# latk/hbetune.rs

Hardware: AMD Instinct MI355X
Metric: GP fit+predict/sec (n=4096,d=8,f64) (higher is better)
Workload: dtype f64; 1 GPU; M: rosenbrock d=8 n=4096 f64, Matern nu=5/2 x constant + white noise; fixed-work fit = 3 L-BFGS runs x 150 lml+gradient evaluations + K^-1, then predict mean+variance at m=1600; evals_per_fit=450, n_not_pd=0, m_candidates=1600, parallelism=replicas x1 (independent fits per GPU, no collective)

## Files before the change

### csrc/dag_kernel.inc.hpp

```cpp

template <typename T, int TA, int TB>
struct DagGeom {
  using C = Cfg<T>;
  static constexpr int NT = 512;
  static constexpr int BK = C::BK;
  static constexpr int SK = BK + 2;
  static constexpr int SMA = TA + 16, SMB = TB + 16;
  static constexpr int LDSA = (TA * SK > BK * SMA) ? TA * SK : BK * SMA;
  static constexpr int LDSB = (TB * SK > BK * SMB) ? TB * SK : BK * SMB;
  static constexpr int NCHA = TA * BK / C::VEC / NT, NCHB = TB * BK / C::VEC / NT;
  static constexpr int WM = 4, WN = 2;
  static constexpr int TMA = TA / WM / 16, TMB = TB / WN / 16;
  static_assert(NCHA >= 1 && NCHB >= 1 && TMA >= 1 && TMB >= 1, "tile too small for 512 threads");
};

constexpr int DAG_LDS_CTL_OFF = (int)((LeafGeom<double>::LDS_BYTES + 15) / 16 * 16);
constexpr int DAG_LDS_BYTES = DAG_LDS_CTL_OFF + 128;
static_assert(DAG_LDS_BYTES <= 163840, "the diagonal block and the control words must fit the CU's LDS");

template <typename T, int TA, int TB, typename PullFn, typename FetchFn>
__device__ __forceinline__ void dag_gemm_tile(int flags, int row0, int col0, int kbeg, int kend, T* __restrict__ W1,
                                              T* __restrict__ W2, T* __restrict__ W3, T* __restrict__ Kinv, int ld, char* smem_raw,
                                              PullFn pull, FetchFn fetch, unsigned long long* inner = nullptr) {
  using C = Cfg<T>;
  using G = DagGeom<T, TA, TB>;
  using vec_t = typename C::vec_t;
  using acc_t = typename C::acc_t;
  constexpr int VEC = C::VEC, BK = G::BK, SK = G::SK, SMA = G::SMA, SMB = G::SMB, NCHA = G::NCHA, NCHB = G::NCHB;
  constexpr int TMA = G::TMA, TMB = G::TMB, NT = G::NT;

  const int akm = (flags & DAGF_AKM) ? 1 : 0, bkm = (flags & DAGF_BKM) ? 1 : 0;
  const T* Ag = (flags & DAGF_A3) ? W3 : ((flags & DAGF_ABUF) ? W2 : W1);
  const T* Bg = (flags & DAGF_B3) ? W3 : ((flags & DAGF_BBUF) ? W2 : W1);
  T* Cg = (flags & DAGF_CKINV) ? Kinv : ((flags & DAGF_C3) ? W3 : ((flags & DAGF_CBUF) ? W2 : W1));
  const int nstages = (kend - kbeg) / BK;

  T* lds = reinterpret_cast<T*>(smem_raw);
  const int t = threadIdx.x, lane = t & 63, wave = t >> 6;
  const int wm = wave >> 1, wn = wave & 1;

  constexpr int CPK = BK / VEC;
  constexpr int RPP_K = NT / CPK;
  constexpr int CPRA = TA / VEC, CPRB = TB / VEC;
  constexpr int RPP_MA = NT / CPRA, RPP_MB = NT / CPRB;
  const int a_r0 = akm ? t / CPRA : t / CPK, a_c0 = akm ? (t % CPRA) * VEC : (t % CPK) * VEC;
  const int b_r0 = bkm ? t / CPRB : t / CPK, b_c0 = bkm ? (t % CPRB) * VEC : (t % CPK) * VEC;
  const int a_rpp = akm ? RPP_MA : RPP_K, b_rpp = bkm ? RPP_MB : RPP_K;
  const int a_lds0 = a_r0 * (akm ? SMA : SK) + a_c0, a_ldsq = a_rpp * (akm ? SMA : SK);
  const int b_lds0 = 2 * G::LDSA + b_r0 * (bkm ? SMB : SK) + b_c0, b_ldsq = b_rpp * (bkm ? SMB : SK);

  const T* pA = Ag + (akm ? (size_t)(kbeg + a_r0) * ld + row0 + a_c0 : (size_t)(row0 + a_r0) * ld + kbeg + a_c0);
  const T* pB = Bg + (bkm ? (size_t)(kbeg + b_r0) * ld + col0 + b_c0 : (size_t)(col0 + b_r0) * ld + kbeg + b_c0);
  const size_t a_step = akm ? (size_t)BK * ld : (size_t)BK, b_step = bkm ? (size_t)BK * ld : (size_t)BK;
  const size_t a_qs = (size_t)a_rpp * ld, b_qs = (size_t)b_rpp * ld;

  vec_t ra0[NCHA], rb0[NCHB], ra1[NCHA], rb1[NCHB];
  auto load_stage = [&](vec_t (&ra)[NCHA], vec_t (&rb)[NCHB]) {
#pragma unroll
    for (int q = 0; q < NCHA; ++q) ra[q] = *reinterpret_cast<const vec_t*>(pA + q * a_qs);
#pragma unroll
    for (int q = 0; q < NCHB; ++q) rb[q] = *reinterpret_cast<const vec_t*>(pB + q * b_qs);
    pA += a_step;
    pB += b_step;
  };
  auto store_stage = [&](int buf, vec_t (&ra)[NCHA], vec_t (&rb)[NCHB]) {
#pragma unroll
    for (int q = 0; q < NCHA; ++q) C::lds_store(lds + buf * G::LDSA + a_lds0 + q * a_ldsq, ra[q]);
#pragma unroll
    for (int q = 0; q < NCHB; ++q) C::lds_store(lds + buf * G::LDSB + b_lds0 + q * b_ldsq, rb[q]);
  };

  acc_t acc[TMA][TMB];
// ... 47 lines not shown
#pragma unroll
      for (int a = 0; a < TMA; ++a)
#pragma unroll
        for (int b = 0; b < TMB; ++b) {
#pragma unroll
          for (int r = 0; r < 4; ++r) tot[a][b][r] += (double)acc[a][b][r];
          acc[a][b] = acc_t{0, 0, 0, 0};
          if constexpr (TA * TB >= 128 * 128) __builtin_amdgcn_sched_barrier(0);
        }
    }
  };

  const int soA = akm ? 1 : SK, skA = akm ? SMA : 1;
  const int soB = bkm ? 1 : SK, skB = bkm ? SMB : 1;
  const int fa0 = (wm * (TA / G::WM) + (lane & 15)) * soA + (lane >> 4) * skA;
  const int fb0 = 2 * G::LDSA + (wn * (TB / G::WN) + (lane & 15)) * soB + (lane >> 4) * skB;

  constexpr int NK = BK / 4;
  T fa[NK][TMA], fb[NK][TMB];
  auto read_frags = [&](int buf, int k4) {
    const int ia = buf * G::LDSA + fa0 + k4 * 4 * skA, ib = buf * G::LDSB + fb0 + k4 * 4 * skB;
#pragma unroll
    for (int a = 0; a < TMA; ++a) fa[k4][a] = lds[ia + a * 16 * soA];
#pragma unroll
    for (int b2 = 0; b2 < TMB; ++b2) fb[k4][b2] = lds[ib + b2 * 16 * soB];
  };
  auto mfma_step = [&](int k4) {
#pragma unroll
    for (int a = 0; a < TMA; ++a)
#pragma unroll
      for (int b2 = 0; b2 < TMB; ++b2) acc[a][b2] = C::mfma(fa[k4][a], fb[k4][b2], acc[a][b2]);
  };
  auto stage = [&](int cur, bool do_load, vec_t (&la)[NCHA], vec_t (&lb)[NCHB], bool do_store, vec_t (&sa)[NCHA],
                   vec_t (&sb)[NCHB], bool has_next) {
    if (do_load) load_stage(la, lb);
    constexpr bool SPLIT_READS = NK >= 8 && TA * TB >= 128 * 128;
    constexpr int KH = SPLIT_READS ? NK / 2 : NK - 1;
#pragma unroll
    for (int k4 = 1; k4 <= KH; ++k4) read_frags(cur, k4);
    if constexpr (SPLIT_READS) {
#pragma unroll
      for (int k4 = 0; k4 + 1 < KH; ++k4) mfma_step(k4);
      __builtin_amdgcn_sched_barrier(0);
#pragma unroll
      for (int k4 = KH + 1; k4 < NK; ++k4) read_frags(cur, k4);
#pragma unroll
      for (int k4 = KH - 1; k4 + 2 < NK; ++k4) mfma_step(k4);
    } else {
#pragma unroll
      for (int k4 = 0; k4 + 2 < NK; ++k4) mfma_step(k4);
    }
    __builtin_amdgcn_sched_barrier(0);
    if (do_store) store_stage(cur ^ 1, sa, sb);
    if (NK >= 2) mfma_step(NK - 2);
    __builtin_amdgcn_sched_barrier(0);
    __syncthreads();
    __builtin_amdgcn_sched_barrier(0);
    if (has_next) read_frags(cur ^ 1, 0);
    mfma_step(NK - 1);
    __builtin_amdgcn_sched_group_barrier(0x100, TMA + TMB, 0);
    __builtin_amdgcn_sched_group_barrier(0x008, TMA * TMB, 0);
    __builtin_amdgcn_sched_barrier(0);
    kabs += BK;
    if (CHUNKED && kabs % F32_CHUNK == 0) flush();
  };
  if (nstages > 0) {
    load_stage(ra0, rb0);
    if (nstages > 1) load_stage(ra1, rb1);
    if constexpr (!PREFETCH_C && !NOACC) {
      if (accum) {
        T cst[TMA][TMB][4];
        const int er0p = row0 + wm * (TA / G::WM), ec0p = col0 + wn * (TB / G::WN) + (lane & 15);
#pragma unroll
        for (int a = 0; a < TMA; ++a)
#pragma unroll
          for (int b = 0; b < TMB; ++b)
#pragma unroll
            for (int r = 0; r < 4; ++r) cst[a][b][r] = Cg[(size_t)(er0p + a * 16 + C::crow(lane, r)) * ld + ec0p + b * 16];
        store_stage(0, ra0, rb0);
        bool stash = true;
        if constexpr (sizeof(T) == 8) {
          if (cinit) {
            stash = false;
#pragma unroll
            for (int a = 0; a < TMA; ++a)
#pragma unroll
              for (int b = 0; b < TMB; ++b)
#pragma unroll
                for (int r = 0; r < 4; ++r) acc[a][b][r] = cst[a][b][r];
          }
        }
        if (stash) {
#pragma unroll
          for (int a = 0; a < TMA; ++a)
#pragma unroll
            for (int b = 0; b < TMB; ++b)
#pragma unroll
              for (int r = 0; r < 4; ++r) lds[STASH_OFF + ((a * TMB + b) * 4 + r) * NT + t] = cst[a][b][r];
        }
      } else {
        store_stage(0, ra0, rb0);
      }
    } else {
      store_stage(0, ra0, rb0);
    }
    __syncthreads();
    read_frags(0, 0);
#ifdef DAG_STAMP_INNER
    unsigned long long st1 = 0;
    if (inner && t == 0) st1 = __builtin_amdgcn_s_memrealtime();
#endif
    int s = 0;
    for (; s + 3 < nstages; s += 2) {
      stage(0, true, ra0, rb0, true, ra1, rb1, true);
      stage(1, true, ra1, rb1, true, ra0, rb0, true);
    }
    const int left = nstages - s;
    if (left <= 2) pull();
    if (left == 1) fetch();
    stage(0, left > 2, ra0, rb0, left > 1, ra1, rb1, left > 1);
    if (left > 2) pull();
    if (left == 2) fetch();
    if (left > 1) stage(1, false, ra1, rb1, left > 2, ra0, rb0, left > 2);
    if (left > 2) {
      fetch();
      stage(0, false, ra0, rb0, false, ra1, rb1, false);
    }
#ifdef DAG_STAMP_INNER
    if (inner && t == 0) *inner = ((st1 & 0xffffffffull) << 32) | (__builtin_amdgcn_s_memrealtime() & 0xffffffffull);
#endif
  } else {
    pull();
    fetch();
  }

  flush();
  const int er0 = row0 + wm * (TA / G::WM), ec0 = col0 + wn * (TB / G::WN) + (lane & 15);
  const bool neg = (flags & DAGF_NEG) != 0;
  T cend[NOACC ? TMA : 1][NOACC ? TMB : 1][4];
  if constexpr (NOACC) {
    if (accum) {
#pragma unroll
      for (int a = 0; a < TMA; ++a)
#pragma unroll
        for (int b = 0; b < TMB; ++b)
#pragma unroll
          for (int r = 0; r < 4; ++r) cend[a][b][r] = Cg[(size_t)(er0 + a * 16 + C::crow(lane, r)) * ld + ec0 + b * 16];
    }
  }
#pragma unroll
  for (int a = 0; a < TMA; ++a)
#pragma unroll
    for (int b = 0; b < TMB; ++b)
#pragma unroll
      for (int r = 0; r < 4; ++r) {
        const int row = er0 + a * 16 + C::crow(lane, r);
        T* p = Cg + (size_t)row * ld + ec0 + b * 16;
        T v;
        if constexpr (CHUNKED) v = (T)tot[a][b][r];
// ... 178 lines not shown
    const int kind = kf & 0xffff, flags = (kf >> 16) & 0xffff;
    const int row0 = __builtin_amdgcn_readfirstlane(ctl[5]), col0 = __builtin_amdgcn_readfirstlane(ctl[6]);
    const int kbeg = __builtin_amdgcn_readfirstlane(ctl[7]), kend = __builtin_amdgcn_readfirstlane(ctl[8]);
    const int sig0 = (__builtin_amdgcn_readfirstlane(ctl[9]) >> 16) & 0xffff, sig12 = __builtin_amdgcn_readfirstlane(ctl[10]);
    const int sig1 = sig12 & 0xffff, sig2 = (sig12 >> 16) & 0xffff;
    const int this_idx = __builtin_amdgcn_readfirstlane(ctl[0]);
    int ndesc = 0, nidx = 0;
    bool pulled = false, fetched = false;
    auto pull = [&]() {
      if (t == 0) nxt = __hip_atomic_fetch_add(g.ctrl, 1, __ATOMIC_RELAXED, __HIP_MEMORY_SCOPE_AGENT);
      pulled = true;
    };
    auto fetch = [&]() {
      if (t < 64) {
        nidx = __builtin_amdgcn_readfirstlane(nxt);
        if (nidx < g.ntasks && t < TASK_DW) ndesc = reinterpret_cast<const int*>(g.tasks + nidx)[t];
      }
      fetched = true;
    };
#ifdef DAG_STAMP_INNER
    unsigned long long* inner_stamp = g.trace ? g.trace + (size_t)this_idx * 5 + 4 : nullptr;
#else
    unsigned long long* inner_stamp = nullptr;
#endif
    if (status == 0) {
      if (kind == DAG_LEAF) {
        dag_leaf_task<T>(W1, W2, g.ld, row0, static_cast<T*>(g.ldiag), g.info, smem_raw, g.leaf_dbg & 16);
      } else if ((flags & DAGF_CKINV) && g.Kinv == nullptr) {
      } else if (kind == DAG_GEMM_128x64) {
        dag_gemm_tile<T, 128, 64>(flags, row0, col0, kbeg, kend, W1, W2, static_cast<T*>(g.W3), static_cast<T*>(g.Kinv), g.ld, smem_raw, pull, fetch, inner_stamp);
      } else if (kind == DAG_GEMM_64x64) {
        dag_gemm_tile<T, 64, 64>(flags, row0, col0, kbeg, kend, W1, W2, static_cast<T*>(g.W3), static_cast<T*>(g.Kinv), g.ld, smem_raw, pull, fetch, inner_stamp);
      } else if (kind == DAG_GEMM_128x128) {
        dag_gemm_tile<T, 128, 128>(flags, row0, col0, kbeg, kend, W1, W2, static_cast<T*>(g.W3), static_cast<T*>(g.Kinv), g.ld, smem_raw, pull, fetch, inner_stamp);
      } else if (kind == DAG_GEMM_32x64) {
        dag_gemm_tile_chain<T>(flags, row0, col0, kbeg, kend, W1, W2, static_cast<T*>(g.W3), g.ld, smem_raw, pull, fetch);
      }
    }
    if (!pulled) pull();
    if (!fetched) fetch();
    if (g.trace && t == 0) g.trace[(size_t)this_idx * 5 + 2] = __builtin_amdgcn_s_memrealtime();
    int* nctl = ctl_base + 16 * (par ^ 1);
    int look_c = 0, look_need = 0, look_inf = 0;
    const bool have_next = t < 64 && nidx < g.ntasks;
    if (have_next) look_issue(ndesc, &look_c, &look_need, &look_inf);
    asm volatile("s_waitcnt vmcnt(0)" ::: "memory");
    if (t < 64) {
      int nstatus = 2, early = 1;
      if (have_next) {
        const bool all_ok = __ballot(look_c < look_need) == 0ull;
        const int inf = __shfl(look_inf, 8, 64);
        if (inf < 0) {
          nstatus = 2;
        } else if (all_ok) {
          __builtin_amdgcn_fence(__ATOMIC_ACQUIRE, "agent");
          nstatus = inf > 0 ? 1 : 0;
          if (g.trace && t == 0) g.trace[(size_t)nidx * 5 + 0] = __builtin_amdgcn_s_memrealtime();
        } else {
          early = 0;
        }
      }
      if (early) {
        if (t < TASK_DW) nctl[4 + t] = ndesc;
        if (t == 0) {
          nctl[0] = nidx;
          nctl[1] = nstatus;
          asm volatile("s_waitcnt vmcnt(0)" ::: "memory");
// ... 44 lines not shown
```

### csrc/engine.hpp

```cpp
#pragma once
#include <hip/hip_runtime_api.h>
#include <cstddef>
#include <cstdint>

namespace hbegp {

constexpr int NB = 128;
constexpr int MAXD = 64;
constexpr int MAXP = MAXD + 2;

struct EvalParams {
  double noise;
  double amp;
  double ell[MAXD];
  unsigned long long seq;
};

struct EvalOut {
  double lml;
  double yalpha;
  double logdet;
  double grad[MAXP];
  int info;
  int n_warn;
// ... 43 lines not shown
  DAG_GEMM_32x64 = 8,
  DAG_GEMM_128x128 = 9,
};
enum : uint16_t {
  DAGF_ABUF = 1,
  DAGF_BBUF = 2,
  DAGF_CBUF = 4,
  DAGF_AKM = 8,
  DAGF_BKM = 16,
  DAGF_NEG = 32,
  DAGF_ACC = 64,
  DAGF_CKINV = 128,
  DAGF_A3 = 256,
  DAGF_B3 = 512,
  DAGF_C3 = 1024,
  DAGF_CINIT = 2048,
};
constexpr int DAG_MAXWAIT = 4;
constexpr int DAG_MAXSIG = 3;
constexpr uint16_t DAG_NOSIG = 0xffff;
struct DagTask {
  uint16_t kind, flags;
  int32_t row0, col0;
  int32_t kbeg, kend;
  uint16_t nwait;
  uint16_t sig[DAG_MAXSIG];
  uint16_t wcnt[DAG_MAXWAIT];
  uint16_t wval[DAG_MAXWAIT];
  uint16_t cost;
  uint16_t pad_[1];
};
static_assert(DAG_MAXSIG == 3, "DagTask::sig has three entries: dword 5 high half, dword 6 low half, dword 6 high half");
static_assert(sizeof(DagTask) == 48, "DagTask layout");
constexpr int DAG_CTRL_WORDS = 4;
constexpr int DAG_INFO_TIMEOUT = -2;
struct DagLaunch {
  const DagTask* tasks;
  int ntasks;
  int* ctrl;
  void* W1;
  void* W2;
  void* W3;
  void* Kinv;
  int ld;
  void* ldiag;
  int* info;
  unsigned long long* trace;
  unsigned long long wait_ticks;
  int leaf_dbg;
};
template <typename T>
void launch_dag(const DagLaunch& g, int nwg, hipStream_t s);
int dag_stage_depth(bool is_f32);

template <typename T>
void launch_gemm(const GemmLaunch& g, int tile, hipStream_t s);

template <typename T>
void launch_kmat(const T* X, const T* rv, int n, int d, int np, int nu2, const EvalParams* P, T* W, const int* info, hipStream_t s,
                 const EvalPrologue* pro = nullptr);

template <typename T>
void launch_leaf(T* W1, T* W2, int ld, int blk, T* ldiag, int* info, hipStream_t s, int dbg = 0);

template <typename T>
void launch_alpha_lml(const T* Xinv, int np, int n, const T* y, const T* ldiag, T* wbuf, double* part, T* alpha,
                      EvalOut* out, const int* info, hipStream_t s, int* ticket = nullptr);

template <typename T>
void launch_gradtrace(const T* X, int n, int d, int np, int nu2, const EvalParams* P, const T* Kinv, const T* alpha,
                      double* part, EvalOut* out, const int* info, hipStream_t s, int* ticket = nullptr, EvalOut* hout = nullptr);
size_t gradtrace_part_elems(int np, int d);

size_t loo_diag_part_elems(int np, int n);
size_t loo_u_part_elems(int np);
template <typename T>
void launch_loo_diag(const T* Xinv, int np, int n, const T* y, const T* alpha, double* part, T* mean, T* var, T* lpd, double* avec,
                     double* sbvec, EvalOut* out, hipStream_t s);
template <typename T>
void launch_loo_uy(const T* Kinv, int np, int n, const double* avec, const double* sbvec, T* Y, double* pu, T* u, hipStream_t s);
template <typename T>
void launch_loo_trace(const T* X, int n, int d, int np, int nu2, const EvalParams* P, const T* Cm, const T* alpha, const T* u,
// ... 176 lines not shown
```

### csrc/hbegp.cpp

```cpp
#include "../include/hbegp.h"

#include <hip/hip_runtime_api.h>

#include <algorithm>
#include <atomic>
#include <queue>
#include <cmath>
#include <cstdarg>
#include <cstdio>
#include <cstdlib>
#include <cstring>
#include <functional>
#include <limits>
#include <memory>
#include <mutex>
#include <numeric>
#include <string>
#include <thread>
#include <type_traits>
#include <vector>

#include "dag_plan.hpp"
#include "engine.hpp"
#include "lbfgsb.hpp"
// ... 664 lines not shown
  bool dag_rl_ = false;
  double dag_gflop_lauum = 0;
  struct DagVariant {
    int nwg = 0;
    std::vector<DagTask*> tasks;
    std::vector<DagTask> host_tasks;
    int nwg_p1 = 0, ntasks_p1 = 0, nwg_kinv = 0, ntasks_kinv = 0;
    std::vector<DagTask*> tasks_p1, tasks_kinv;
    std::vector<DagTask> host_tasks_p1, host_tasks_kinv;
  };
  std::vector<DagVariant> dag_var;
  std::unique_ptr<std::atomic<int>[]> busy_slots_;
  int dag_ntasks = 0, dag_nwg = 0;
  int dag_nvar_ = 1, dag_ncrowd_ = 0;
  int dag_nshare_ = 0;
  int share_hyst_ = SLOT_SHARE_HYSTERESIS;
  int slot_maxeval_ = 0;
  std::vector<int> share_force_;
  std::vector<char> balance_dev_;
  std::unique_ptr<std::atomic<int>[]> slot_running_, slot_done_;
  mutable std::atomic<int> not_alone_{0};
  unsigned long long dag_wait_ticks_ = 200000000ull;
  size_t dag_ctrl_bytes = 0;
  int dag_ctrl_regions_ = 1;
  double dag_gflop = 0;
  bool adhoc_ = false;
  bool small_ = false;
  bool like_fit_ = false;
  bool lazy_ = false;
  std::function<std::shared_ptr<const DagPlan>(int, bool, int)> plan_for_;
  bool hostio_ = true;
  bool eval_published() const { return hostio_ && !small_; }
  int leaf_dbg_ = 0;

  struct Pooled { int dev; void* p; size_t bytes; };
  std::vector<Pooled> pooled_;
  template <typename U>
  U* palloc(int dev, size_t count) {
    bool fresh = false;
    const size_t bytes = std::max<size_t>(16, sizeof(U) * count);
    void* q = g_pool.get(dev, bytes, &fresh);
    pooled_.push_back({dev, q, bytes});
    return static_cast<U*>(q);
  }

  Problem(hbegp_ctx* c, const T* X, const T* y, int n_, int d_, double nu, int n_slots_, bool single_shot = false, bool like_fit = false,
          bool lazy_fit = false, const double* rv = nullptr) {
    try {
      adhoc_ = single_shot;
      like_fit_ = like_fit;
      lazy_ = lazy_fit && env_int("HBEGP_LAZY_GRAD", 1) != 0;
      init(c, X, y, n_, d_, nu, n_slots_, rv);
    } catch (...) {
      release();
      throw;
    }
  }

  void init(hbegp_ctx* c, const T* X, const T* y, int n_, int d_, double nu, int n_slots_, const double* rv) {
    ctx = c; n = n_; d = d_; np = round_up(n_, NB); n_slots = n_slots_;
    nu2 = std::isinf(nu) ? 0 : (int)std::lround(2 * nu);
    is_f32 = sizeof(T) == 4;
    leaf_dbg_ = env_int("HBEGP_LEAF_DBG", 0) & 16;
    small_ = np == NB && d <= SMALL_EVAL_MAXD && env_int("HBEGP_SMALL", 1) != 0;
    hostio_ = env_int("HBEGP_HOSTIO", 1) != 0;
    lazy_ = lazy_ && eval_published() && !adhoc_;
    const size_t nn = (size_t)np * np;
    Xd.assign(c->devs.size(), nullptr);
    yd.assign(c->devs.size(), nullptr);
    rvd.assign(c->devs.size(), nullptr);
    std::vector<T> rv_t;
    if (rv) rv_t.assign(rv, rv + n_);
    slots.resize(c->devs.size());
    for (size_t di = 0; di < c->devs.size(); ++di) {
      HIPCHECK(hipSetDevice(c->devs[di]));
      slots[di].resize(n_slots);
      for (auto& s : slots[di]) {
        s.dev = c->devs[di];
        s.stream = g_stream_pool.get(s.dev);
      }
      hipStream_t st0 = slots[di][0].stream;
      Xd[di] = palloc<T>(c->devs[di], (size_t)n * d);
      yd[di] = palloc<T>(c->devs[di], np);
      HIPCHECK(hipMemsetAsync(yd[di], 0, sizeof(T) * np, st0));
      HIPCHECK(hipMemcpyAsync(Xd[di], X, sizeof(T) * (size_t)n * d, hipMemcpyHostToDevice, st0));
      HIPCHECK(hipMemcpyAsync(yd[di], y, sizeof(T) * n, hipMemcpyHostToDevice, st0));
      if (rv) {
        rvd[di] = palloc<T>(c->devs[di], n);
        HIPCHECK(hipMemcpyAsync(rvd[di], rv_t.data(), sizeof(T) * n, hipMemcpyHostToDevice, st0));
      }
      for (auto& s : slots[di]) {
        bool fresh1 = false, fresh2 = false, fk = false;
        s.W1 = static_cast<T*>(g_pool.get(s.dev, sizeof(T) * nn, &fresh1));
        s.W2 = static_cast<T*>(g_pool.get(s.dev, sizeof(T) * nn, &fresh2));
        for (int b = 0; b < 2; ++b) s.Kinv[b] = static_cast<T*>(g_pool.get(s.dev, sizeof(T) * nn, &fk));
        HIPCHECK(hipMemsetAsync(s.W2, 0, sizeof(T) * nn, st0));
// ... 355 lines not shown
    if (!s.dag_ctrl) return;
    std::vector<int> ctrl(dag_ctrl_bytes / sizeof(int));
    if (hipMemcpyAsync(ctrl.data(), s.dag_ctrl + (s.dag_part == 2 ? dag_ctrl_bytes / sizeof(int) : 0), dag_ctrl_bytes, hipMemcpyDeviceToHost, s.stream) != hipSuccess || hipStreamSynchronize(s.stream) != hipSuccess) return;
    const int row = ctrl[1] - 1;
    const DagVariant& var = dag_var[s.dag_variant];
    const int ntasks_here = s.dag_part == 1 ? var.ntasks_p1 : (s.dag_part == 2 ? var.ntasks_kinv : dag_ntasks);
    fprintf(stderr, "task queue timeout: queue head %d of %d, first task that gave up: %d\n", ctrl[0], ntasks_here, row);
    const std::vector<DagTask>& host_tasks = s.dag_part == 1 ? var.host_tasks_p1 : (s.dag_part == 2 ? var.host_tasks_kinv : var.host_tasks);
    if (row >= 0 && row < (int)host_tasks.size()) {
      const DagTask& t = host_tasks[row];
      fprintf(stderr, "  kind %d flags %x row0 %d col0 %d k [%d, %d) waits:", t.kind, t.flags, t.row0, t.col0, t.kbeg, t.kend);
      for (int w = 0; w < t.nwait; ++w) fprintf(stderr, " c%d=%d/%d", t.wcnt[w], ctrl[DAG_CTRL_WORDS + t.wcnt[w]], t.wval[w]);
      fprintf(stderr, "\n");
    }
    (void)hipGetLastError();
  }

  void launch_queue(Slot<T>& s, size_t di, T* Kinv, PhaseTimer* tm, int part = 0) {
    if (part != 2 && !s.ctrl_cleared) HIPCHECK(hipMemsetAsync(s.dag_ctrl, 0, dag_ctrl_regions_ * dag_ctrl_bytes, s.stream));
    if (part != 2) s.ctrl_cleared = false;
    DagLaunch g{};
    const DagVariant& var = dag_var[s.dag_variant];
    g.tasks = var.tasks[di]; g.ntasks = dag_ntasks; g.ctrl = s.dag_ctrl;
    int nwg = var.nwg;
    s.dag_part = part;
    if (part == 1) { g.tasks = var.tasks_p1[di]; g.ntasks = var.ntasks_p1; nwg = var.nwg_p1; }
    if (part == 2) { g.tasks = var.tasks_kinv[di]; g.ntasks = var.ntasks_kinv; nwg = var.nwg_kinv; g.ctrl = s.dag_ctrl + dag_ctrl_bytes / sizeof(int); }
    g.W1 = s.W1; g.W2 = s.W2; g.ld = np; g.ldiag = s.ldiag; g.info = &s.dOut->info;
    g.W3 = s.W3;
    g.Kinv = (dag_lauum_ && part != 1) ? Kinv : nullptr;
    g.trace = s.dag_trace;
    g.wait_ticks = dag_wait_ticks_;
    g.leaf_dbg = leaf_dbg_;
    if (tm) tm->begin(PhaseTimer::DAG, 0, part == 2 ? dag_gflop_lauum : (g.Kinv ? dag_gflop : dag_gflop - dag_gflop_lauum));
    launch_dag<T>(g, nwg, s.stream);
    if (tm) tm->end();
  }

  void small_eval(Slot<T>& s, size_t di, int target, int mode) {
    SmallEval g{};
    g.X = Xd[di]; g.y = yd[di]; g.n = n; g.d = d;
    g.W2 = s.W2; g.ldiag = s.ldiag; g.Kinv = s.Kinv[target]; g.alpha = s.alpha[target]; g.out = s.dOut; g.mode = mode;
    g.P = s.hP; g.hout = s.hOut;
    launch_small_eval<T>(g, rvd[di], nu2, s.stream);
  }

  enum EvalMode { EVAL_LML_KINV = 0, EVAL_FULL = 1, EVAL_LML_ONLY = 2, EVAL_GRAD_ONLY = 3 };

  void enqueue_eval(Slot<T>& s, size_t di, int target, int mode, PhaseTimer* tm) {
    const int* info = &s.dOut->info;
    const bool want_grad = mode == EVAL_FULL || mode == EVAL_GRAD_ONLY;
    if (mode == EVAL_GRAD_ONLY) {
      if (dag_ && dag_lauum_) launch_queue(s, di, s.Kinv[target], tm, 2);
      else eval_gemms(s, s.Kinv[target], scheduled(s, di, tm, (int)scheds[di].size() - 1), leaf_step(s, tm), [] {}, 2);
      const bool fuse_grad = (np / 64) * (np / 64 + 1) / 2 <= 512;
      if (tm) tm->begin(PhaseTimer::GRAD);
      launch_gradtrace<T>(Xd[di], n, d, np, nu2, s.dP, s.Kinv[target], s.alpha[target], s.part_g, s.dOut, info, s.stream,
                          fuse_grad ? s.tickets + 1 : nullptr, fuse_grad ? s.hOut : nullptr);
      if (tm) tm->end();
      if (!fuse_grad) launch_publish_out(s.dOut, s.hOut, s.dP, s.stream);
      s.published = true;
      CHECK_LAUNCHES();
      return;
    }
    const int part = mode == EVAL_LML_ONLY ? 1 : 0;
    if (small_) {
// ... 3866 lines not shown
int hbegp_debug_dag_replay(int nblocks, int bk, int small_h, int nwg, int order_wg, int fine, int big128, int which, int workers,
                           int* ntasks, int* tasks, int cap, double* out, char* err, int errlen) {
  if (nblocks < 1 || (bk != 16 && bk != 32) || small_h < 0 || nwg < 1 || which < 0 || which > 2 || !ntasks || workers < 0)
    return fail(HBEGP_EINVAL, "bad argument");
  GUARD_BEGIN
  DagBuilder builder(bk, small_h, nwg, (fine & 1) != 0, order_wg);
  builder.set_rl_progressive((fine & 16) != 0);
  builder.set_big128(big128 != 0, big128 >= 2);
  builder.set_rl(32, 1, (fine & 32) == 0, true);
  DagPlan plan = builder.build(0, nblocks, which != 1, (fine & 8) != 0);
  if (which == 2) plan = dag_plan_kinv_only(plan);
  const std::string why = plan.tasks.empty() ? std::string("no tasks") : dag_plan_validate(plan, nblocks);
  *ntasks = (int)plan.tasks.size();
  if (tasks)
    for (int i = 0; i < std::min(cap, (int)plan.tasks.size()); ++i) {
      const DagTask& t = plan.tasks[i];
      int* v = tasks + (size_t)18 * i;
      v[0] = t.kind; v[1] = t.flags; v[2] = t.row0; v[3] = t.col0; v[4] = t.kbeg; v[5] = t.kend; v[6] = t.nwait;
      for (int w = 0; w < DAG_MAXWAIT; ++w) { v[7 + w] = w < t.nwait ? t.wcnt[w] : 0; v[11 + w] = w < t.nwait ? t.wval[w] : 0; }
      for (int q = 0; q < DAG_MAXSIG; ++q) v[15 + q] = t.sig[q];
    }
  if (out) {
    const DagReplay r = workers > 0 ? dag_plan_replay(plan, workers) : DagReplay();
    double acc128 = 0;
    for (const DagTask& t : plan.tasks)
      if (t.kind == DAG_GEMM_128x128 && (t.flags & DAGF_ACC)) acc128 += t.cost * 0.1;
    out[0] = r.makespan_us; out[1] = r.wait_us; out[2] = r.busy_us; out[3] = plan.sim_us; out[4] = plan.crit_us; out[5] = acc128;
  }
  if (err && errlen > 0) snprintf(err, (size_t)errlen, "%s", why.c_str());
  return why.empty() ? HBEGP_OK : fail(HBEGP_EINVAL, "%s", why.c_str());
  GUARD_END
}

int hbegp_debug_dag_order_wg(int queue, int share, int nwg, int even_wg, int nblocks, int n_slots) {
  return dag_default_order_wg(queue, share, nwg, even_wg, nblocks, n_slots);
}

int hbegp_debug_lbfgs_replay(int n, const double* x0, const double* lo, const double* hi, int maxeval, int memory, int fixed_work,
                             int count, const double* f, const double* g, double* requested, int* n_requested) {
  if (n < 1 || n > LBFGS_MAXN || count < 0 || !x0 || !lo || !hi || !requested || !n_requested || (count > 0 && (!f || !g)))
    return fail(HBEGP_EINVAL, "bad argument");
  GUARD_BEGIN
  return lbfgs_replay_impl(n, x0, lo, hi, maxeval, memory, fixed_work, count, f, g, requested, nullptr, nullptr, nullptr, n_requested);
  GUARD_END
}

int hbegp_debug_dag_plan(int nblocks, int bk, int small_h, int nwg, int fine, int* ntasks, int* ncounters, int* nleaf,
                         double* gflop, double* crit_us, double* sim_us, char* err, int errlen) {
  if (nblocks < 1 || (bk != 16 && bk != 32) || small_h < 0 || nwg < 0) return fail(HBEGP_EINVAL, "bad argument");
  GUARD_BEGIN
  DagBuilder builder(bk, small_h, nwg, (fine & 1) != 0);
  builder.set_rl_progressive((fine & 16) != 0);
  builder.set_big128(getenv("HBEGP_DAG_BIG128") && atoi(getenv("HBEGP_DAG_BIG128")) != 0, getenv("HBEGP_DAG_BIG128") && atoi(getenv("HBEGP_DAG_BIG128")) >= 2);
  if (fine & 2) return fail(HBEGP_EINVAL, "fine bit 1 (kernel-matrix / reduction tasks in the queue) no longer exists");
  DagPlan plan = builder.build(0, nblocks, (fine & 4) != 0, (fine & 8) != 0);
  if (const char* fault = getenv("HBEGP_DAG_TEST_FAULT")) {
    int a = 0, b = 0;
    if (sscanf(fault, "drop:%d", &a) == 1 && a >= 0 && a < (int)plan.tasks.size() && plan.tasks[a].nwait > 0) {
      DagTask& t = plan.tasks[a];
      for (int w = 1; w < t.nwait; ++w) { t.wcnt[w - 1] = t.wcnt[w]; t.wval[w - 1] = t.wval[w]; }
      t.nwait--;
    } else if (sscanf(fault, "move:%d:%d", &a, &b) == 2 && a >= 0 && b >= 0 && a < (int)plan.tasks.size() && b < (int)plan.tasks.size()) {
      const DagTask t = plan.tasks[a];
      plan.tasks.erase(plan.tasks.begin() + a);
      plan.tasks.insert(plan.tasks.begin() + b, t);
    }
// ... 34 lines not shown
```

### hbetune_rs_amd/_lib.py

```python
import ctypes as C
import os

import numpy as np

HERE = os.path.dirname(os.path.abspath(__file__))
LIB_PATH = os.environ.get("HBEGP_LIB") or os.path.join(HERE, "libhbegp.so")

OK, NOT_PD, ALL_FAILED = 0, 1, 2
EINVAL, EHIP, ENODEV, ENOMEM = -1, -2, -3, -4
PATHS_MAX_FEATURES, PATHS_MAX_PATHS = 16384, 1024
CEI_MAX_CONSTRAINTS = 8
MES_MAX_SAMPLES = 1024
EHVI_ND_MAX_BOXES = 1048576
STATS_MAX_RUNS = 16


class HbegpError(RuntimeError):
    def __init__(self, code, msg):
        super().__init__(f"hbegp error {code}: {msg}")
        self.code = code


class FitOptions(C.Structure):

# ... 139 lines not shown
    "hbegp_paths_eval_f64": (C.c_int, [_vp, _dp, C.c_int, C.c_int, _dp, _dp]),
    "hbegp_paths_eval_f32": (C.c_int, [_vp, _fp, C.c_int, C.c_int, _fp, _fp]),
    "hbegp_paths_minimize_f64": (C.c_int, [_vp, _dp, C.c_int, _dp, _dp, C.c_int, _dp, _dp, _ip]),
    "hbegp_paths_minimize_f32": (C.c_int, [_vp, _fp, C.c_int, _dp, _dp, C.c_int, _fp, _dp, _ip]),
    "hbegp_paths_info": (C.c_int, [_vp, _ip, _ip, _ip, _ip, _ip]),
    "hbegp_paths_release": (None, [_vp]),
    "hbegp_debug_paths_phases": (C.c_int, [C.c_int, _dp]),
    "hbegp_debug_posterior_phases": (C.c_int, [C.c_int, _dp]),
    "hbegp_debug_batch_select_phases": (C.c_int, [C.c_int, _dp]),
    "hbegp_debug_kg_phases": (C.c_int, [C.c_int, _dp]),
    "hbegp_debug_nei_phases": (C.c_int, [C.c_int, _dp]),
    "hbegp_debug_sens_phases": (C.c_int, [C.c_int, _dp]),
    "hbegp_debug_ehvi_phases": (C.c_int, [C.c_int, _dp]),
    "hbegp_debug_ehvi_nd_phases": (C.c_int, [C.c_int, _dp]),
    "hbegp_debug_cei_phases": (C.c_int, [C.c_int, _dp]),
    "hbegp_debug_lcei_phases": (C.c_int, [C.c_int, _dp]),
    "hbegp_debug_mes_phases": (C.c_int, [C.c_int, _dp]),
    "hbegp_debug_cb_phases": (C.c_int, [C.c_int, _dp]),
    "hbegp_debug_pool_poisoned": (C.c_int, [C.POINTER(C.c_longlong), C.POINTER(C.c_longlong)]),
    "hbegp_model_info": (C.c_int, [_vp, _ip, _ip, _ip, _dp, _dp]),
    "hbegp_model_get_f64": (C.c_int, [_vp, _dp, _dp, _dp]),
    "hbegp_model_get_f32": (C.c_int, [_vp, _dp, _fp, _fp]),
    "hbegp_model_debug_params": (C.c_int, [_vp, _dp]),
    "hbegp_model_retain": (None, [_vp]),
    "hbegp_model_release": (None, [_vp]),
    "hbegp_debug_lbfgs_replay": (C.c_int, [C.c_int, _dp, _dp, _dp, C.c_int, C.c_int, C.c_int, C.c_int, _dp, _dp, _dp, _ip]),
    "hbegp_last_fit_stats": (C.c_int, [C.POINTER(FitStats)]),
    "hbegp_debug_lbfgs_decisions": (C.c_int, [C.c_int, _dp, _dp, _dp, C.c_int, C.c_int, C.c_int, C.c_int, _dp, _dp, _dp, _ip, _ip, _ip, _ip]),
    "hbegp_debug_dag_queues": (C.c_int, [C.c_int, C.c_int, C.c_int, C.c_int, C.c_int, C.c_int, C.c_int, _ip, _ip, C.c_int, C.c_char_p,
                                         C.c_int]),
    "hbegp_debug_dag_replay": (C.c_int, [C.c_int, C.c_int, C.c_int, C.c_int, C.c_int, C.c_int, C.c_int, C.c_int, C.c_int, _ip, _ip,
                                         C.c_int, _dp, C.c_char_p, C.c_int]),
    "hbegp_debug_dag_order_wg": (C.c_int, [C.c_int, C.c_int, C.c_int, C.c_int, C.c_int, C.c_int]),
    "hbegp_debug_slot_shares": (C.c_int, [C.c_int, _ip, _ip, _ip, C.c_int, _ip, C.c_int, C.c_int, _ip, _ip]),
    "hbegp_debug_fits_in_flight": (C.c_int, [C.c_int]),
    "hbegp_debug_dag_plan": (C.c_int, [C.c_int, C.c_int, C.c_int, C.c_int, C.c_int, _ip, _ip, _ip, _dp, _dp, _dp, C.c_char_p,
                                       C.c_int]),
    "hbegp_minimize_by_gradient": (C.c_double, [OBJECTIVE_FN, _vp, _dp, _dp, _dp, C.c_int, C.c_int]),
    "hbegp_problem_create_rv_f64": (C.c_int, [_vp, _dp, _dp, _dp, C.c_int, C.c_int, C.c_double, C.c_int, C.POINTER(_vp)]),
    "hbegp_problem_create_rv_f32": (C.c_int, [_vp, _fp, _fp, _dp, C.c_int, C.c_int, C.c_double, C.c_int, C.POINTER(_vp)]),
    "hbegp_fit_rv_f64": (C.c_int, [_vp, _dp, _dp, _dp, C.c_int, C.c_int, C.c_double, _dp, _dp, _dp, _dp, C.c_int,
                                   C.POINTER(FitOptions), _dp, _dp, C.POINTER(_vp)]),
    "hbegp_fit_rv_f32": (C.c_int, [_vp, _fp, _fp, _dp, C.c_int, C.c_int, C.c_double, _dp, _dp, _dp, _dp, C.c_int,
                                   C.POINTER(FitOptions), _dp, _dp, C.POINTER(_vp)]),
    "hbegp_fit_loo_rv_f64": (C.c_int, [_vp, _dp, _dp, _dp, C.c_int, C.c_int, C.c_double, _dp, _dp, _dp, _dp, C.c_int,
                                       C.POINTER(FitOptions), _dp, _dp, C.POINTER(_vp)]),
    "hbegp_fit_loo_rv_f32": (C.c_int, [_vp, _fp, _fp, _dp, C.c_int, C.c_int, C.c_double, _dp, _dp, _dp, _dp, C.c_int,
                                       C.POINTER(FitOptions), _dp, _dp, C.POINTER(_vp)]),
    "hbegp_extend_rv_f64": (C.c_int, [_vp, _dp, _dp, _dp, C.c_int, C.c_int, C.c_double, _dp, _dp, _dp, C.POINTER(_vp)]),
    "hbegp_extend_rv_f32": (C.c_int, [_vp, _fp, _fp, _dp, C.c_int, C.c_int, C.c_double, _dp, _dp, _dp, C.POINTER(_vp)]),
    "hbegp_extend_from_rv_f64": (C.c_int, [_vp, _vp, _dp, _dp, _dp, C.c_int, C.POINTER(_vp), _ip]),
    "hbegp_extend_from_rv_f32": (C.c_int, [_vp, _vp, _fp, _fp, _dp, C.c_int, C.POINTER(_vp), _ip]),
    "hbegp_model_row_variance": (C.c_int, [_vp, _dp]),
}

_lib = None


def load():
    global _lib
    if _lib is not None:
        return _lib
    if not os.path.exists(LIB_PATH):
        raise ImportError(
            f"{LIB_PATH} is missing: build it with `python -c 'import __graft_entry__ as g; g.build()'` or `make`. "
            "hbetune_rs_amd has no CPU fallback."
# ... 41 lines not shown
```

### include/hbegp.h

```cpp
#ifndef HBEGP_H
#define HBEGP_H

#include <stddef.h>

#ifdef __cplusplus
extern "C" {
#endif

#define HBEGP_VERSION 200

enum {
  HBEGP_OK = 0,
  HBEGP_NOT_PD = 1,
  HBEGP_ALL_FAILED = 2,
  HBEGP_EINVAL = -1,
  HBEGP_EHIP = -2,
  HBEGP_ENODEV = -3,
  HBEGP_ENOMEM = -4
};

typedef struct hbegp_ctx hbegp_ctx;
typedef struct hbegp_problem hbegp_problem;
typedef struct hbegp_model hbegp_model;

// ... 238 lines not shown

int hbegp_model_info(const hbegp_model* model, int* n, int* d, int* is_f32, double* nu, double* lml);
int hbegp_model_get_f64(hbegp_model* model, double* theta, double* alpha, double* kinv);
int hbegp_model_get_f32(hbegp_model* model, double* theta, float* alpha, float* kinv);
void hbegp_model_retain(hbegp_model* model);
void hbegp_model_release(hbegp_model* model);

typedef double (*hbegp_objective_fn)(const double* x, double* grad, void* user);
double hbegp_minimize_by_gradient(hbegp_objective_fn f, void* user, double* x, const double* lo, const double* hi,
                                  int n, int maxeval);

int hbegp_problem_debug_get_f64(hbegp_problem* prob, int dev, int slot, int which, double* out);
int hbegp_problem_debug_get_f32(hbegp_problem* prob, int dev, int slot, int which, float* out);

int hbegp_model_debug_params(hbegp_model* model, double* out);

int hbegp_debug_dag_plan(int nblocks, int bk, int small_h, int nwg, int fine, int* ntasks, int* ncounters, int* nleaf,
                         double* gflop, double* crit_us, double* sim_us, char* err, int errlen);

int hbegp_debug_lbfgs_replay(int n, const double* x0, const double* lo, const double* hi, int maxeval, int memory, int fixed_work,
                             int count, const double* f, const double* g, double* requested, int* n_requested);

int hbegp_debug_lbfgs_decisions(int n, const double* x0, const double* lo, const double* hi, int maxeval, int memory, int fixed_work,
                                int count, const double* f, const double* g, double* requested, int* trial, int* accepted, int* took,
                                int* n_requested);

int hbegp_debug_dag_queues(int nblocks, int bk, int small_h, int nwg, int fine, int big128, int which, int* ntasks, int* tasks, int cap,
                           char* err, int errlen);

int hbegp_debug_dag_replay(int nblocks, int bk, int small_h, int nwg, int order_wg, int fine, int big128, int which, int workers,
                           int* ntasks, int* tasks, int cap, double* out, char* err, int errlen);
int hbegp_debug_dag_order_wg(int queue, int share, int nwg, int even_wg, int nblocks, int n_slots);

int hbegp_debug_slot_shares(int n_slots, const int* running, const int* done, const int* maxeval, int hysteresis, int* share, int even_wg,
                            int cus, int* lead_wg, int* lag_wg);
int hbegp_debug_fits_in_flight(int device_id);

int hbegp_debug_pool_poisoned(long long* blocks, long long* bytes);
int hbegp_debug_posterior_phases(int enable, double* phase_ms);
int hbegp_debug_batch_select_phases(int enable, double* phase_ms);
int hbegp_debug_kg_phases(int enable, double* phase_ms);
int hbegp_debug_nei_phases(int enable, double* phase_ms);
int hbegp_debug_ehvi_phases(int enable, double* phase_ms);
int hbegp_debug_ehvi_nd_phases(int enable, double* phase_ms);
int hbegp_debug_ehvi_boxes(const double* front, int P, int n_obj, const double* ref, int* thr_count, double* thr, int thr_cap,
                           int* n_boxes, int* boxes, int box_cap);
int hbegp_debug_cei_phases(int enable, double* phase_ms);
int hbegp_debug_lcei_phases(int enable, double* phase_ms);
int hbegp_debug_mes_phases(int enable, double* phase_ms);
int hbegp_debug_cb_phases(int enable, double* phase_ms);
int hbegp_debug_sens_phases(int enable, double* phase_ms);
int hbegp_debug_qei_phases(int enable, double* phase_ms);

int hbegp_debug_loo_phases(int enable, double* phase_ms);

#define HBEGP_PATHS_MAX_FEATURES 16384
#define HBEGP_PATHS_MAX_PATHS 1024
typedef struct hbegp_paths hbegp_paths;
int hbegp_paths_create_f64(hbegp_model* model, const double* omega0, const double* phase, const double* w, const double* eps, int F, int S,
                           hbegp_paths** paths);
int hbegp_paths_create_f32(hbegp_model* model, const float* omega0, const float* phase, const float* w, const float* eps, int F, int S,
                           hbegp_paths** paths);
int hbegp_paths_eval_f64(hbegp_paths* paths, const double* Xs, int m, int per_path, double* f, double* df);
int hbegp_paths_eval_f32(hbegp_paths* paths, const float* Xs, int m, int per_path, float* f, float* df);
int hbegp_paths_minimize_f64(hbegp_paths* paths, const double* starts, int R, const double* lo, const double* hi, int maxeval,
                             double* x_best, double* f_best, int* n_evals);
// ... 11 lines not shown
```

Measured before the change: 2.006 fit+predict/s.

## Skip MFMA work on structurally zero triangular halves in 128x128 DAG GEMM tiles

For 128x128 GEMM tiles reading from the triangular W2 buffer, it computes per-wave leading and trailing K stages where that wave's 64-row half of A or B is structurally zero, and skips the LDS fragment reads and MFMAs for those stages while still keeping loads, stores and barriers. Wave-to-quadrant mapping is permuted (wn = wave xor wave>>2) so that the skipped work is spread more evenly across SIMDs. The aim is to remove redundant FLOPs in the triangular inverse/LAUUM GEMMs. It is controlled by an env flag that defaults to on, and it adds branchy stage loops and a dependence on the zero structure being exact.

```diff
diff --git a/csrc/dag_kernel.inc.hpp b/csrc/dag_kernel.inc.hpp
--- a/csrc/dag_kernel.inc.hpp
+++ b/csrc/dag_kernel.inc.hpp
@@ -18,10 +18,10 @@
 constexpr int DAG_LDS_BYTES = DAG_LDS_CTL_OFF + 128;
 static_assert(DAG_LDS_BYTES <= 163840, "the diagonal block and the control words must fit the CU's LDS");
 
-template <typename T, int TA, int TB, typename PullFn, typename FetchFn>
+template <typename T, int TA, int TB, bool PAIRED = true, typename PullFn, typename FetchFn>
 __device__ __forceinline__ void dag_gemm_tile(int flags, int row0, int col0, int kbeg, int kend, T* __restrict__ W1,
                                               T* __restrict__ W2, T* __restrict__ W3, T* __restrict__ Kinv, int ld, char* smem_raw,
-                                              PullFn pull, FetchFn fetch, unsigned long long* inner = nullptr) {
+                                              PullFn pull, FetchFn fetch, unsigned long long* inner = nullptr, bool zero_skip = false) {
   using C = Cfg<T>;
   using G = DagGeom<T, TA, TB>;
   using vec_t = typename C::vec_t;
@@ -37,7 +37,20 @@
 
   T* lds = reinterpret_cast<T*>(smem_raw);
   const int t = threadIdx.x, lane = t & 63, wave = t >> 6;
-  const int wm = wave >> 1, wn = wave & 1;
+  constexpr bool BIG = TA == 128 && TB == 128;
+  const int wm = wave >> 1, wn = (BIG && PAIRED) ? ((wave ^ (wave >> 2)) & 1) : (wave & 1);
+  int lead_w = 0, trail_w = 0, lead_wg = 0, trail_wg = 0;
+  if constexpr (BIG) {
+    if (zero_skip) {
+      const DagZeroHalf z = dag_zero_halves(flags, row0, col0, kbeg, kend, BK);
+      const int wu = __builtin_amdgcn_readfirstlane(wave);
+      const int ha = wu >> 2, hb = PAIRED ? ((wu ^ (wu >> 2)) & 1) : (wu & 1);
+      lead_w = max(ha ? z.lead[0][1] : z.lead[0][0], hb ? z.lead[1][1] : z.lead[1][0]);
+      trail_w = max(ha ? z.trail[0][1] : z.trail[0][0], hb ? z.trail[1][1] : z.trail[1][0]);
+      lead_wg = max(max(z.lead[0][0], z.lead[0][1]), max(z.lead[1][0], z.lead[1][1]));
+      trail_wg = max(max(z.trail[0][0], z.trail[0][1]), max(z.trail[1][0], z.trail[1][1]));
+    }
+  }
 
   constexpr int CPK = BK / VEC;
   constexpr int RPP_K = NT / CPK;
@@ -151,32 +164,34 @@
       for (int b2 = 0; b2 < TMB; ++b2) acc[a][b2] = C::mfma(fa[k4][a], fb[k4][b2], acc[a][b2]);
   };
   auto stage = [&](int cur, bool do_load, vec_t (&la)[NCHA], vec_t (&lb)[NCHB], bool do_store, vec_t (&sa)[NCHA],
-                   vec_t (&sb)[NCHB], bool has_next) {
+                   vec_t (&sb)[NCHB], bool has_next, bool skip) __attribute__((always_inline)) {
     if (do_load) load_stage(la, lb);
     constexpr bool SPLIT_READS = NK >= 8 && TA * TB >= 128 * 128;
     constexpr int KH = SPLIT_READS ? NK / 2 : NK - 1;
-#pragma unroll
-    for (int k4 = 1; k4 <= KH; ++k4) read_frags(cur, k4);
-    if constexpr (SPLIT_READS) {
-#pragma unroll
-      for (int k4 = 0; k4 + 1 < KH; ++k4) mfma_step(k4);
-      __builtin_amdgcn_sched_barrier(0);
-#pragma unroll
-      for (int k4 = KH + 1; k4 < NK; ++k4) read_frags(cur, k4);
-#pragma unroll
-      for (int k4 = KH - 1; k4 + 2 < NK; ++k4) mfma_step(k4);
-    } else {
-#pragma unroll
-      for (int k4 = 0; k4 + 2 < NK; ++k4) mfma_step(k4);
+    if (!skip) {
+#pragma unroll
+      for (int k4 = 1; k4 <= KH; ++k4) read_frags(cur, k4);
+      if constexpr (SPLIT_READS) {
+#pragma unroll
+        for (int k4 = 0; k4 + 1 < KH; ++k4) mfma_step(k4);
+        __builtin_amdgcn_sched_barrier(0);
+#pragma unroll
+        for (int k4 = KH + 1; k4 < NK; ++k4) read_frags(cur, k4);
+#pragma unroll
+        for (int k4 = KH - 1; k4 + 2 < NK; ++k4) mfma_step(k4);
+      } else {
+#pragma unroll
+        for (int k4 = 0; k4 + 2 < NK; ++k4) mfma_step(k4);
+      }
     }
     __builtin_amdgcn_sched_barrier(0);
     if (do_store) store_stage(cur ^ 1, sa, sb);
-    if (NK >= 2) mfma_step(NK - 2);
+    if (NK >= 2 && !skip) mfma_step(NK - 2);
     __builtin_amdgcn_sched_barrier(0);
     __syncthreads();
     __builtin_amdgcn_sched_barrier(0);
     if (has_next) read_frags(cur ^ 1, 0);
-    mfma_step(NK - 1);
+    if (!skip) mfma_step(NK - 1);
     __builtin_amdgcn_sched_group_barrier(0x100, TMA + TMB, 0);
     __builtin_amdgcn_sched_group_barrier(0x008, TMA * TMB, 0);
     __builtin_amdgcn_sched_barrier(0);
@@ -230,20 +245,33 @@
     if (inner && t == 0) st1 = __builtin_amdgcn_s_memrealtime();
 #endif
     int s = 0;
-    for (; s + 3 < nstages; s += 2) {
-      stage(0, true, ra0, rb0, true, ra1, rb1, true);
-      stage(1, true, ra1, rb1, true, ra0, rb0, true);
+    auto skips = [&](int si) { return BIG && (si < lead_w || si >= nstages - trail_w); };
+    if constexpr (BIG) {
+      for (; s < lead_wg && s + 3 < nstages; s += 2) {
+        stage(0, true, ra0, rb0, true, ra1, rb1, true, skips(s));
+        stage(1, true, ra1, rb1, true, ra0, rb0, true, skips(s + 1));
+      }
+    }
+    for (; s + 3 < nstages - trail_wg; s += 2) {
+      stage(0, true, ra0, rb0, true, ra1, rb1, true, false);
+      stage(1, true, ra1, rb1, true, ra0, rb0, true, false);
+    }
+    if constexpr (BIG) {
+      for (; s + 3 < nstages; s += 2) {
+        stage(0, true, ra0, rb0, true, ra1, rb1, true, skips(s));
+        stage(1, true, ra1, rb1, true, ra0, rb0, true, skips(s + 1));
+      }
     }
     const int left = nstages - s;
     if (left <= 2) pull();
     if (left == 1) fetch();
-    stage(0, left > 2, ra0, rb0, left > 1, ra1, rb1, left > 1);
+    stage(0, left > 2, ra0, rb0, left > 1, ra1, rb1, left > 1, skips(s));
     if (left > 2) pull();
     if (left == 2) fetch();
-    if (left > 1) stage(1, false, ra1, rb1, left > 2, ra0, rb0, left > 2);
+    if (left > 1) stage(1, false, ra1, rb1, left > 2, ra0, rb0, left > 2, skips(s + 1));
     if (left > 2) {
       fetch();
-      stage(0, false, ra0, rb0, false, ra1, rb1, false);
+      stage(0, false, ra0, rb0, false, ra1, rb1, false, skips(s + 2));
     }
 #ifdef DAG_STAMP_INNER
     if (inner && t == 0) *inner = ((st1 & 0xffffffffull) << 32) | (__builtin_amdgcn_s_memrealtime() & 0xffffffffull);
@@ -488,7 +516,7 @@
       } else if (kind == DAG_GEMM_64x64) {
         dag_gemm_tile<T, 64, 64>(flags, row0, col0, kbeg, kend, W1, W2, static_cast<T*>(g.W3), static_cast<T*>(g.Kinv), g.ld, smem_raw, pull, fetch, inner_stamp);
       } else if (kind == DAG_GEMM_128x128) {
-        dag_gemm_tile<T, 128, 128>(flags, row0, col0, kbeg, kend, W1, W2, static_cast<T*>(g.W3), static_cast<T*>(g.Kinv), g.ld, smem_raw, pull, fetch, inner_stamp);
+        dag_gemm_tile<T, 128, 128>(flags, row0, col0, kbeg, kend, W1, W2, static_cast<T*>(g.W3), static_cast<T*>(g.Kinv), g.ld, smem_raw, pull, fetch, inner_stamp, g.zero_skip != 0);
       } else if (kind == DAG_GEMM_32x64) {
         dag_gemm_tile_chain<T>(flags, row0, col0, kbeg, kend, W1, W2, static_cast<T*>(g.W3), g.ld, smem_raw, pull, fetch);
       }
diff --git a/csrc/engine.hpp b/csrc/engine.hpp
--- a/csrc/engine.hpp
+++ b/csrc/engine.hpp
@@ -99,6 +99,38 @@
 };
 static_assert(DAG_MAXSIG == 3, "DagTask::sig has three entries: dword 5 high half, dword 6 low half, dword 6 high half");
 static_assert(sizeof(DagTask) == 48, "DagTask layout");
+
+#if defined(__HIPCC__) || defined(__CUDACC__)
+#define HBEGP_HD __host__ __device__
+#else
+#define HBEGP_HD
+#endif
+struct DagZeroHalf {
+  int lead[2][2], trail[2][2];
+};
+HBEGP_HD inline DagZeroHalf dag_zero_halves(int flags, int row0, int col0, int kbeg, int kend, int bk) {
+  DagZeroHalf z = {{{0, 0}, {0, 0}}, {{0, 0}, {0, 0}}};
+  const int nst = (kend - kbeg) / bk;
+  if (nst <= 0) return z;
+  for (int side = 0; side < 2; ++side) {
+    const bool in_w2 = side == 0 ? ((flags & DAGF_ABUF) != 0 && (flags & DAGF_A3) == 0) : ((flags & DAGF_BBUF) != 0 && (flags & DAGF_B3) == 0);
+    if (!in_w2) continue;
+    const bool km = (flags & (side == 0 ? DAGF_AKM : DAGF_BKM)) != 0;
+    for (int h = 0; h < 2; ++h) {
+      const int r = (side == 0 ? row0 : col0) + 64 * h;
+      if (km) {
+        const int c = r > kbeg ? (r - kbeg) / bk : 0;
+        z.lead[side][h] = c < nst ? c : nst;
+      } else {
+        const int d = r + 64 - kbeg;
+        const int first = d > 0 ? (d + bk - 1) / bk : 0;
+        z.trail[side][h] = first < nst ? nst - first : 0;
+      }
+    }
+  }
+  return z;
+}
+
 constexpr int DAG_CTRL_WORDS = 4;
 constexpr int DAG_INFO_TIMEOUT = -2;
 struct DagLaunch {
@@ -115,6 +147,7 @@
   unsigned long long* trace;
   unsigned long long wait_ticks;
   int leaf_dbg;
+  int zero_skip;
 };
 template <typename T>
 void launch_dag(const DagLaunch& g, int nwg, hipStream_t s);
diff --git a/csrc/hbegp.cpp b/csrc/hbegp.cpp
--- a/csrc/hbegp.cpp
+++ b/csrc/hbegp.cpp
@@ -720,6 +720,7 @@
   bool hostio_ = true;
   bool eval_published() const { return hostio_ && !small_; }
   int leaf_dbg_ = 0;
+  bool zero_skip_ = true;
 
   struct Pooled { int dev; void* p; size_t bytes; };
   std::vector<Pooled> pooled_;
@@ -750,6 +751,7 @@
     nu2 = std::isinf(nu) ? 0 : (int)std::lround(2 * nu);
     is_f32 = sizeof(T) == 4;
     leaf_dbg_ = env_int("HBEGP_LEAF_DBG", 0) & 16;
+    zero_skip_ = env_int("HBEGP_DAG_ZERO_SKIP", 1) != 0;
     small_ = np == NB && d <= SMALL_EVAL_MAXD && env_int("HBEGP_SMALL", 1) != 0;
     hostio_ = env_int("HBEGP_HOSTIO", 1) != 0;
     lazy_ = lazy_ && eval_published() && !adhoc_;
@@ -1171,6 +1173,7 @@
     g.trace = s.dag_trace;
     g.wait_ticks = dag_wait_ticks_;
     g.leaf_dbg = leaf_dbg_;
+    g.zero_skip = zero_skip_ ? 1 : 0;
     if (tm) tm->begin(PhaseTimer::DAG, 0, part == 2 ? dag_gflop_lauum : (g.Kinv ? dag_gflop : dag_gflop - dag_gflop_lauum));
     launch_dag<T>(g, nwg, s.stream);
     if (tm) tm->end();
@@ -5103,6 +5106,14 @@
   GUARD_END
 }
 
+int hbegp_debug_dag_zero_halves(int flags, int row0, int col0, int kbeg, int kend, int bk, int* out) {
+  if (bk < 1 || !out) return fail(HBEGP_EINVAL, "bad argument");
+  const DagZeroHalf z = dag_zero_halves(flags, row0, col0, kbeg, kend, bk);
+  for (int side = 0; side < 2; ++side)
+    for (int h = 0; h < 2; ++h) { out[2 * side + h] = z.lead[side][h]; out[4 + 2 * side + h] = z.trail[side][h]; }
+  return HBEGP_OK;
+}
+
 int hbegp_debug_dag_order_wg(int queue, int share, int nwg, int even_wg, int nblocks, int n_slots) {
   return dag_default_order_wg(queue, share, nwg, even_wg, nblocks, n_slots);
 }
diff --git a/hbetune_rs_amd/_lib.py b/hbetune_rs_amd/_lib.py
--- a/hbetune_rs_amd/_lib.py
+++ b/hbetune_rs_amd/_lib.py
@@ -195,6 +195,7 @@
     "hbegp_debug_dag_replay": (C.c_int, [C.c_int, C.c_int, C.c_int, C.c_int, C.c_int, C.c_int, C.c_int, C.c_int, C.c_int, _ip, _ip,
                                          C.c_int, _dp, C.c_char_p, C.c_int]),
     "hbegp_debug_dag_order_wg": (C.c_int, [C.c_int, C.c_int, C.c_int, C.c_int, C.c_int, C.c_int]),
+    "hbegp_debug_dag_zero_halves": (C.c_int, [C.c_int, C.c_int, C.c_int, C.c_int, C.c_int, C.c_int, _ip]),
     "hbegp_debug_slot_shares": (C.c_int, [C.c_int, _ip, _ip, _ip, C.c_int, _ip, C.c_int, C.c_int, _ip, _ip]),
     "hbegp_debug_fits_in_flight": (C.c_int, [C.c_int]),
     "hbegp_debug_dag_plan": (C.c_int, [C.c_int, C.c_int, C.c_int, C.c_int, C.c_int, _ip, _ip, _ip, _dp, _dp, _dp, C.c_char_p,
diff --git a/include/hbegp.h b/include/hbegp.h
--- a/include/hbegp.h
+++ b/include/hbegp.h
@@ -294,6 +294,8 @@
                            int* ntasks, int* tasks, int cap, double* out, char* err, int errlen);
 int hbegp_debug_dag_order_wg(int queue, int share, int nwg, int even_wg, int nblocks, int n_slots);
 
+int hbegp_debug_dag_zero_halves(int flags, int row0, int col0, int kbeg, int kend, int bk, int* out);
+
 int hbegp_debug_slot_shares(int n_slots, const int* running, const int* done, const int* maxeval, int hysteresis, int* share, int even_wg,
                             int cus, int* lead_wg, int* lag_wg);
 int hbegp_debug_fits_in_flight(int device_id);
```

New measurement: 2.039 fit+predict/s, median of 6. 1.02x the previous value.
